# mrperkett/genome-kmers

Hardware: AMD Instinct MI355X
Metric: sorted 31-mers/sec end-to-end on 3.1 Gb synthetic genome; % HBM roofline (higher is better)
Workload: dtype u64

## Files before the change

genome-kmers_amd/csrc/gkm_msd.hip:

```cpp
#include <algorithm>
#include <cstdio>
#include <cstdlib>
#include <cstring>

#include "gkm_canon.h"
#include "gkm_internal.h"
#include "gkm_partition.h"
#include "gkm_swar.h"

namespace gkm {

constexpr int kGR = 8;
constexpr int kGRadix = 1 << kGR;
#ifndef GKM_PT
#define GKM_PT 1024
#endif
#ifndef GKM_PI
#define GKM_PI 11
#endif
constexpr int kPT = GKM_PT, kPI = GKM_PI;
constexpr int kWideL0 = 11, kWT = 512, kWI = 36;
constexpr int kPTile = kPT * kPI;
constexpr int kChunkTiles = 256;
constexpr int kBT = 512, kBI = 8, kBR = 8;
constexpr int kBT2 = 1024, kBR2 = 10;
constexpr int kBlockMax = kBT2 * kBI;
constexpr int kLocal = 6;
constexpr int kTiny = 8;
constexpr int kSmall = 24;
#ifndef GKM_WAVE_OCC8
#define GKM_WAVE_OCC8 4
#endif
constexpr int kWaveOcc4 = 6, kWaveOcc8 = GKM_WAVE_OCC8, kWaveOcc16 = 3;
#ifndef GKM_WAVE_R8
#define GKM_WAVE_R8 9
#endif
constexpr int kWaveR4 = 8, kWaveR8 = GKM_WAVE_R8, kWaveR16 = 10;
constexpr int kSmallLate = 96;
constexpr int kMaxLevels = 16;

__constant__ uint8_t c_code4_msd[256];
static bool g_msd_tables = false;

static hipError_t msd_tables() {
    if (g_msd_tables) return hipSuccess;
// ... 1120 lines not shown
            tile_hist[(f + i + u) * RADIX + d] = run;
            run += v[u];
        }
    }
    for (; i < nt; ++i) {
        const uint32_t v = tile_hist[(f + i) * RADIX + d];
        tile_hist[(f + i) * RADIX + d] = run;
        run += v;
    }
}

__device__ __forceinline__ uint32_t wave_append(bool flag, uint32_t *counter, int lane) {
    const uint64_t m = __ballot(flag);
    if (!m) return 0;
    const int leader = __ffsll((unsigned long long)m) - 1;
    uint32_t base = 0;
    if (lane == leader) base = atomicAdd(counter, (uint32_t)__popcll(m));
    base = __shfl(base, leader);
    const uint64_t lt_mask = (lane == 0) ? 0ull : (~0ull >> (64 - lane));
    return base + (uint32_t)__popcll(m & lt_mask);
}

enum { kCtrBig = 0, kCtrDone = 1, kCtrLoc = 2, kLists = kCtrLoc + kLocal, kCtrNbCopy = kLists, kCtrN = 8 + 2 };
enum { kSumTiles = kLists, kSumChunks = kLists + 1, kSumN = kLists + 2 };

__host__ __device__ inline uint32_t tiles_of(uint32_t len, uint32_t tile) { return (len + tile - 1) / tile; }
__host__ __device__ inline uint32_t chunks_of(uint32_t len, uint32_t tile, uint32_t ctiles) {
    return (tiles_of(len, tile) + ctiles - 1) / ctiles;
}

struct Lists {
    uint32_t *nb_start, *nb_len;
    uint32_t *dn_start, *dn_len;
    uint8_t *dn_par;
    uint2 *loc[kLocal];
    uint64_t *nb_pref;
    uint64_t *loc_pref[kLocal];
};

constexpr uint64_t kCompact = 1ull << 63;

__device__ __forceinline__ uint64_t compact_key(uint64_t pref, int hi, int B, uint32_t dig, uint32_t low) {
    const int rem = B - hi;
    return ((pref & ~kCompact) << rem) | ((uint64_t)dig << (rem - 8)) | (uint64_t)low;
}

__host__ __device__ constexpr uint32_t local_cap(int cls) {
// ... 22 lines not shown
        const uint2 le = local_entry(st, size, hi, parity);
        gmem(reinterpret_cast<uint64_t *>(L.loc[l - kCtrLoc]))[at] = ((uint64_t)le.y << 32) | le.x;
        if (L.loc_pref[l - kCtrLoc]) gmem(L.loc_pref[l - kCtrLoc])[at] = pref;
    }
}

__device__ __forceinline__ void route(uint32_t st, uint32_t size, int hi, int B, int parity, bool allow_big,
                                      const Lists &L, uint32_t *ctr, int lane) {
    const int li = size >= 1 ? list_of(size, hi, B, allow_big) : -1;
#pragma unroll
    for (int l = 0; l < kLists; ++l) {
        const uint32_t at = wave_append(li == l, &ctr[l], lane);
        if (li == l) put_entry(L, l, at, st, size, hi, parity);
    }
}

constexpr int kClassT = 1024;

__global__ __launch_bounds__(kClassT) void classify_kernel(const uint32_t *__restrict__ seg_base,
                                                           const uint32_t *__restrict__ seg_cnt, uint64_t nsub, int hi,
                                                           int B, int parity, Lists L, uint32_t *__restrict__ ctr,
                                                           unsigned long long *__restrict__ sums, uint32_t min_size,
                                                           const uint64_t *__restrict__ ppref, int pw, int compact,
                                                           uint32_t tile, uint32_t ctiles) {
    constexpr int NW = kClassT / 64;
    __shared__ uint32_t s_cnt[kLists][NW];
    __shared__ uint32_t s_elems[kLists][NW];
    __shared__ uint32_t s_base[kLists];
    __shared__ uint32_t s_tc[2][NW];
    const int tid = threadIdx.x, lane = tid & 63, wave = tid >> 6;
    const uint64_t i = (uint64_t)blockIdx.x * kClassT + tid;
    const uint32_t size = i < nsub ? seg_cnt[i] : 0, st = i < nsub ? seg_base[i] : 0;
    const int li = size >= min_size ? list_of(size, hi, B, true) : -1;
    bool f[kLists];
#pragma unroll
    for (int l = 0; l < kLists; ++l) f[l] = li == l;
    uint32_t below[kLists];
#pragma unroll
    for (int l = 0; l < kLists; ++l) {
        const uint64_t m = __ballot(f[l]);
        below[l] = lanes_below(m);
        uint32_t e = f[l] ? size : 0;
#pragma unroll
        for (int off = 32; off >= 1; off >>= 1) e += __shfl_xor(e, off);
        if (lane == 0) {
            s_cnt[l][wave] = (uint32_t)__popcll(m);
            s_elems[l][wave] = e;
        }
    }
    {
        uint32_t tl = li == kCtrBig ? tiles_of(size, tile) : 0, ch = li == kCtrBig ? chunks_of(size, tile, ctiles) : 0;
#pragma unroll
        for (int off = 32; off >= 1; off >>= 1) {
            tl += __shfl_xor(tl, off);
            ch += __shfl_xor(ch, off);
        }
        if (lane == 0) {
            s_tc[0][wave] = tl;
            s_tc[1][wave] = ch;
        }
    }
    __syncthreads();
    if (tid >= 64 && tid < 66) {
        unsigned long long t = 0;
        for (int w = 0; w < NW; ++w) t += s_tc[tid - 64][w];
        if (t) atomicAdd(&sums[kSumTiles + tid - 64], t);
    }
    if (tid < kLists) {
        uint32_t tot = 0;
        unsigned long long el = 0;
        for (int w = 0; w < NW; ++w) {
            tot += s_cnt[tid][w];
            el += s_elems[tid][w];
        }
        s_base[tid] = tot ? atomicAdd(&ctr[tid], tot) : 0;
        if (el) atomicAdd(&sums[tid], el);
    }
    __syncthreads();
    uint32_t at[kLists];
#pragma unroll
    for (int l = 0; l < kLists; ++l) {
        uint32_t pre = s_base[l];
        for (int w = 0; w < wave; ++w) pre += s_cnt[l][w];
        at[l] = pre + below[l];
    }
    uint64_t pref = 0;
// ... 841 lines not shown
}

__global__ __launch_bounds__(256) void uniform_flag_kernel(const uint32_t *__restrict__ bst,
                                                           const uint32_t *__restrict__ blen,
                                                           const uint64_t *__restrict__ keys,
                                                           uint32_t *__restrict__ mixed,
                                                           const uint32_t *__restrict__ nb_dev = nullptr,
                                                           uint32_t *__restrict__ nb_copy = nullptr) {
    if (nb_copy && blockIdx.x == 0 && blockIdx.y == 0 && threadIdx.x == 0) *nb_copy = *nb_dev;
    if (nb_dev && blockIdx.x >= *nb_dev) return;
    const uint64_t st = bst[blockIdx.x];
    const uint32_t len = blen[blockIdx.x];
    const uint64_t k0 = keys[st];
    uint64_t acc = 0;
    for (uint32_t e = blockIdx.y * 256 + threadIdx.x; e < len; e += gridDim.y * 256) acc |= keys[st + e] ^ k0;
    if (__syncthreads_or(acc != 0) && threadIdx.x == 0) atomicOr(&mixed[blockIdx.x], 1u);
}

__global__ __launch_bounds__(256) void route_uniform_kernel(const uint32_t *__restrict__ bst,
                                                            const uint32_t *__restrict__ blen,
                                                            const uint64_t *__restrict__ bpref, uint32_t nb,
                                                            const uint32_t *__restrict__ mixed, Lists L, int parity,
                                                            uint32_t *__restrict__ ctr,
                                                            unsigned long long *__restrict__ sums, uint32_t tile,
                                                            uint32_t ctiles, const uint32_t *__restrict__ nb_dev = nullptr) {
    if (nb_dev) nb = *nb_dev;
    for (uint32_t b = blockIdx.x * 256 + threadIdx.x; b < nb; b += gridDim.x * 256) {
        if (mixed[b]) {
            const uint32_t at = atomicAdd(&ctr[kCtrBig], 1u);
            put_entry(L, kCtrBig, at, bst[b], blen[b], 0, parity, bpref ? bpref[b] : 0);
            atomicAdd(&sums[kCtrBig], (unsigned long long)blen[b]);
            atomicAdd(&sums[kSumTiles], (unsigned long long)tiles_of(blen[b], tile));
            atomicAdd(&sums[kSumChunks], (unsigned long long)chunks_of(blen[b], tile, ctiles));
        } else {
            put_entry(L, kCtrDone, atomicAdd(&ctr[kCtrDone], 1u), bst[b], blen[b], 0, parity);
        }
    }
}

__global__ __launch_bounds__(256) void done_copy_kernel(const uint32_t *__restrict__ dn_start,
                                                        const uint32_t *__restrict__ dn_len,
                                                        const uint8_t *__restrict__ dn_par, const uint32_t *__restrict__ v1,
                                                        uint32_t *__restrict__ v0, const uint64_t *__restrict__ k1,
                                                        uint64_t *__restrict__ k0, uint8_t *__restrict__ heads) {
    const uint32_t s = blockIdx.x;
    const uint64_t st = dn_start[s];
    const uint32_t len = dn_len[s];
    const bool copy = dn_par[s];
    for (uint32_t i = blockIdx.y * 256 + threadIdx.x; i < len; i += gridDim.y * 256) {
        if (copy) v0[st + i] = v1[st + i];
        if (copy && k1) k0[st + i] = k1[st + i];
        heads[st + i] = i == 0;
    }
}

template <int BITS>
// ... 532 lines not shown
    int expand_big(int out) {
        if (cur_fmt != Fmt::Compact || nbig == 0) return GK_OK;
        hipLaunchKernelGGL(expand_compact_kernel, dim3(nbig, bucket_split(nbig)), dim3(256), 0, c->stream, big_start[cur_big],
                           big_len[cur_big], big_pref[cur_big], compact_hi, B, nd, c->keys[out], c->vals[out]);
        GK_TRY_HIP(c, hipGetLastError());
        return GK_OK;
    }

    int classify(uint64_t nsub, int hi, int parity, int bigsel, const uint32_t *base = nullptr,
                 const uint32_t *cnt = nullptr, uint32_t min_size = 1, const uint64_t *ppref = nullptr, int pw = 0,
                 int compact = 0, bool read = true) {
        if (!base) base = seg_base;
        if (!cnt) cnt = seg_cnt;
        for (int k = 0; k < kLocal; ++k)
            GK_TRY_HIP(c, grow_keep(c, kLocName[k][0], nloc[k] + nsub, nloc[k], &loc[k][0]));
        for (int k = 0; k < kLocal; ++k)
            GK_TRY_HIP(c, grow_keep(c, kLocPrefName[k], nloc[k] + nsub, nloc[k], &loc_pref[k]));
        if (int rc = grow_done(nsub)) return rc;
        GK_TRY_HIP(c, hipMemsetAsync(ctr + kCtrBig, 0, 4, c->stream));
        GK_TRY_HIP(c, hipMemsetAsync(sums, 0, 8 * kSumN, c->stream));
        timer_begin(c, "msd_classify", &slot);
        hipLaunchKernelGGL(classify_kernel, dim3((unsigned)((nsub + kClassT - 1) / kClassT)), dim3(kClassT), 0,
                           c->stream, base, cnt, nsub, hi, B, parity, lists(0, bigsel), ctr, sums, min_size, ppref, pw,
                           compact, (uint32_t)kPTile, ctiles);
        GK_TRY_HIP(c, hipGetLastError());
        timer_end(c, slot);
        return read ? classify_counts() : GK_OK;
    }

    int classify_counts() {
        int r = read_ctr();
        if (r != GK_OK) return r;
        for (int k = 0; k < kLocal; ++k) {
            nloc[k] = h[kCtrLoc + k];
            loc_elems[k] += hs[kCtrLoc + k];
        }
        ndone = h[kCtrDone];
        nbig = h[kCtrBig];
        big_elems = hs[kCtrBig];
        return GK_OK;
    }

    int route_uniform(int out, uint32_t nb, bool dev_count) {
        const uint32_t *nb_dev = dev_count ? ctr + kCtrBig : nullptr;
        uint32_t *nb_copy = dev_count ? ctr + kCtrNbCopy : nullptr;
        const unsigned split = bucket_split(nb);
        if (dev_count && cur_fmt == Fmt::Compact)
            hipLaunchKernelGGL(expand_compact_kernel, dim3(nb, split), dim3(256), 0, c->stream, big_start[cur_big],
                               big_len[cur_big], big_pref[cur_big], compact_hi, B, nd, c->keys[out], c->vals[out],
                               nb_dev);
        uint32_t *mixed;
        GK_TRY_HIP(c, scratch(c, "uni_mixed", nb, &mixed));
        GK_TRY_HIP(c, hipMemsetAsync(mixed, 0, 4ull * nb, c->stream));
        hipLaunchKernelGGL(uniform_flag_kernel, dim3(nb, split), dim3(256), 0, c->stream, big_start[cur_big],
                           big_len[cur_big], c->keys[out], mixed, nb_dev, nb_copy);
        if (!dev_count)
            if (int rc = grow_done(nb)) return rc;
        GK_TRY_HIP(c, hipMemsetAsync(ctr + kCtrBig, 0, 4, c->stream));
        GK_TRY_HIP(c, hipMemsetAsync(sums + kCtrBig, 0, 8, c->stream));
        GK_TRY_HIP(c, hipMemsetAsync(sums + kSumTiles, 0, 16, c->stream));
        hipLaunchKernelGGL(route_uniform_kernel, dim3(grid256_min1(nb)), dim3(256), 0, c->stream, big_start[cur_big],
                           big_len[cur_big], big_pref[cur_big], nb, mixed, lists(0, cur_big ^ 1), out, ctr, sums,
                           (uint32_t)kPTile, ctiles, nb_copy);
        GK_TRY_HIP(c, hipGetLastError());
        cur_big ^= 1;
        if (dev_count) return classify_counts();
        int r = read_ctr();
        if (r != GK_OK) return r;
        ndone = h[kCtrDone];
        nbig = h[kCtrBig];
        big_elems = hs[kCtrBig];
        return GK_OK;
    }

    bool few_big_elems(int level, uint64_t elems) const {
        return level >= 1 && elems * 64 <= std::max<uint64_t>(c->n, 1);
    }

    static bool reads(Fmt in, Fmt out) {
        switch (in) {
        case Fmt::Pairs: return out == Fmt::Compact;
        case Fmt::PackedL0: return out == Fmt::Pairs;
        default: return true;
        }
    }
    bool has_digits() const { return cur_fmt != Fmt::KeyStart; }

    template <int R>
    void level_launch(int hi, int nw, const uint32_t *t_start, const uint32_t *t_count, uint64_t T,
                      const uint64_t *kin, const uint32_t *vin, int out, bool count, Fmt ofmt) {
        if (count) {
            if (has_digits())
                hipLaunchKernelGGL(msd_count_nd_kernel<R>, dim3((unsigned)T), dim3(256), 0, c->stream, t_start,
                                   t_count, nd, tile_hist);
            else
                hipLaunchKernelGGL(msd_count_kernel<R>, dim3((unsigned)T), dim3(256), 0, c->stream, t_start, t_count,
                                   dig_at(B, hi, R), kin, tile_hist);
            return;
        }
        if (ofmt == Fmt::Compact) {
            const int rem = B - hi - R;
            NextDigits ndg{dig_at(B, hi + R, 8), nd};
            ndg.lowmask = (uint32_t)((1ull << (rem - 8)) - 1);
            if (cur_fmt == Fmt::Pairs)
                hipLaunchKernelGGL((msd_pipe_kernel<kPT, kPI, R, 4, true, 0, true>), dim3(pgrid), dim3(kPT), 0,
                                   c->stream, t_start, t_count, dig_at(B, hi, R), tile_hist, kin, vin, c->keys[out],
                                   c->vals[out], (uint32_t)T, n, ndg, lo16, c79_shi);
            else
                hipLaunchKernelGGL((msd_pipe_kernel<kPT, kPI, R, 4, true>), dim3(pgrid), dim3(kPT), 0, c->stream,
                                   t_start, t_count, dig_at(B, hi, R), tile_hist, kin, vin, c->keys[out],
                                   c->vals[out], (uint32_t)T, n, ndg);
            return;
        }
        if (ofmt == Fmt::Pairs) {
            NextDigits ndg{dig_at(B, hi + R, nw), nd};
            ndg.out16 = lo16;
            ndg.pshi = c79_shi;
            if (cur_fmt == Fmt::PackedL0) {
                ndg.in8 = nd_l0;
                hipLaunchKernelGGL((msd_pipe_kernel<kPT, kPI, R, 5, true, 0, 2>), dim3(pgrid), dim3(kPT), 0, c->stream,
                                   t_start, t_count, dig_at(B, hi, R), tile_hist, kin, vin, c->keys[out], c->vals[out],
                                   (uint32_t)T, n, ndg, lo16_l0, p88_shi);
                return;
            }
            hipLaunchKernelGGL((msd_pipe_kernel<kPT, kPI, R, 5, true>), dim3(pgrid), dim3(kPT), 0, c->stream, t_start,
                               t_count, dig_at(B, hi, R), tile_hist, kin, vin, c->keys[out], c->vals[out],
                               (uint32_t)T, n, ndg);
            return;
        }
        const NextDigits ndg{dig_at(B, hi + R, nw), nd};
        if (ofmt == Fmt::KeyStartDigit)
            hipLaunchKernelGGL((msd_pipe_kernel<kPT, kPI, R, 0, true>), dim3(pgrid), dim3(kPT), 0, c->stream, t_start,
                               t_count, dig_at(B, hi, R), tile_hist, kin, vin, c->keys[out], c->vals[out],
                               (uint32_t)T, n, ndg);
        else
            hipLaunchKernelGGL((msd_pipe_kernel<kPT, kPI, R, 0, false>), dim3(pgrid), dim3(kPT), 0, c->stream,
                               t_start, t_count, dig_at(B, hi, R), tile_hist, kin, vin, c->keys[out], c->vals[out],
                               (uint32_t)T, n, ndg);
    }

    void level_dispatch(int level, int hi, const uint32_t *t_start, const uint32_t *t_count, uint64_t T,
                        const uint64_t *kin, const uint32_t *vin, int out, bool count, Fmt ofmt) {
        const int w = width(level), nw = width(level + 1);
        if (w == 8) level_launch<8>(hi, nw, t_start, t_count, T, kin, vin, out, count, ofmt);
        else if (w == 7) level_launch<7>(hi, nw, t_start, t_count, T, kin, vin, out, count, ofmt);
        else level_launch<6>(hi, nw, t_start, t_count, T, kin, vin, out, count, ofmt);
    }

    Fmt level_format(int level, int hi, uint64_t elems, uint64_t nseg) const {
        const bool digits = nseg == 0 || (elems / nseg >> width(level)) >= (uint64_t)kBlockMax;
        const int rem = B - hi - width(level);
        if (phase == 0 && !digits && rem >= 9 && rem <= 40 && width(level + 1) == 8 && !no_compact())
            return Fmt::Compact;
        const uint64_t next_mean = nseg ? (elems / nseg >> width(level)) >> width(level + 1) : 0;
        const int rem2 = rem - width(level + 1);
        const bool force = opt("GKM_TEST_PAIRS") != nullptr;
        if (allow_c79 && cur_fmt != Fmt::Pairs && phase == 0 && rem >= 33 && rem <= 48 && !no_compact() &&
            (force || (digits && next_mean < (uint64_t)kBlockMax && rem2 >= 9 && rem2 <= 40 &&
                       width(level + 2) == 8 && width(level + 1) == 8)))
            return Fmt::Pairs;
        return digits ? Fmt::KeyStartDigit : Fmt::KeyStart;
    }

    int level_pass(int level, int hi, const uint32_t *t_start, const uint32_t *t_count, uint64_t T, uint64_t C,
                   const uint32_t *s_cfirst, const uint32_t *s_nchunks, const uint32_t *s_start, uint64_t nseg,
                   const uint64_t *kin, const uint32_t *vin, int out) {
        timer_begin(c, has_digits() ? "msd_count_nd" : "msd_count", &slot);
        timer_units(c, slot, big_elems);
        level_dispatch(level, hi, t_start, t_count, T, kin, vin, out, true, cur_fmt);
        GK_TRY_HIP(c, hipGetLastError());
        timer_end(c, slot);
        int rc = scan_offsets(width(level), C, s_cfirst, s_nchunks, s_start, nseg);
        if (rc != GK_OK) return rc;
        GK_TRY_HIP(c, scratch(c, "msd_nd", n + 64, &nd));
        const Fmt ofmt = level_format(level, hi, big_elems, nseg);
        compact_hi = hi + width(level);
        const int rem = B - hi - width(level);
        if (ofmt == Fmt::Pairs) {
            c79_shi = 64 - rem;
            GK_TRY_HIP(c, scratch(c, "msd_lo16", n + 64, &lo16));
        }
        if (!reads(cur_fmt, ofmt)) {
            if (cur_fmt == Fmt::PackedL0) {
                if (int rc = p88_detach()) return rc;
                hipLaunchKernelGGL(expand_p88_kernel, dim3((unsigned)nseg, bucket_split(nseg)), dim3(256), 0,
                                   c->stream, big_start[cur_big], big_len[cur_big], big_pref[cur_big], hi, B, p88_shi,
                                   const_cast<uint64_t *>(kin), lo16_l0, nd_l0, const_cast<uint32_t *>(vin));
            } else {
                hipLaunchKernelGGL(expand_pair_kernel, dim3((unsigned)nseg, bucket_split(nseg)), dim3(256), 0,
                                   c->stream, big_start[cur_big], big_len[cur_big], big_pref[cur_big], hi, B, c79_shi,
                                   const_cast<uint64_t *>(kin), lo16, const_cast<uint32_t *>(vin));
            }
            GK_TRY_HIP(c, hipGetLastError());
            cur_fmt = Fmt::KeyStartDigit;
        }
        timer_begin(c, ofmt == Fmt::Compact ? kPassNamesC[level & 7] : ofmt == Fmt::Pairs ? kPassNamesP[level & 7]
                                                                                          : kPassNames[level & 7],
                    &slot);
        timer_units(c, slot, big_elems);
        level_dispatch(level, hi, t_start, t_count, T, kin, vin, out, false, ofmt);
        GK_TRY_HIP(c, hipGetLastError());
        timer_end(c, slot);
        cur_fmt = ofmt;
        return GK_OK;
    }

    int expand_pair_locals(const uint64_t (&before)[kLocal], int out) {
        for (int k = 0; k < kLocal; ++k) {
            if (nloc[k] <= before[k]) continue;
            hipLaunchKernelGGL(expand_pair_list_kernel, dim3((unsigned)(nloc[k] - before[k])), dim3(256), 0,
                               c->stream, loc[k][0], loc_pref[k], (uint32_t)before[k], B, c79_shi, c->keys[out], lo16,
                               c->vals[out]);
            GK_TRY_HIP(c, hipGetLastError());
        }
        return GK_OK;
    }

    int first_level_from_pieces(const uint64_t *kin, const uint32_t *vin, const uint64_t *poff, const uint64_t *plen,
                                const uint32_t *pbucket, uint32_t np, int level = 1, int hi = kGR) {
        std::vector<uint32_t> ts, tc, cf, cn, scf, snc, sst;
        std::vector<uint64_t> spf;
        uint64_t out_base = 0;
        for (uint32_t i = 0; i < np;) {
            uint32_t j = i;
            uint64_t tot = 0;
            const uint64_t tile0 = ts.size();
            while (j < np && pbucket[j] == pbucket[i]) {
                for (uint64_t o = 0; o < plen[j]; o += kPTile) {
                    ts.push_back((uint32_t)(poff[j] + o));
                    tc.push_back((uint32_t)std::min<uint64_t>(kPTile, plen[j] - o));
                }
                tot += plen[j];
                ++j;
            }
            if (tot > 0) {
                const uint64_t nt = ts.size() - tile0;
                scf.push_back((uint32_t)cf.size());
                for (uint64_t t = 0; t < nt; t += ctiles) {
                    cf.push_back((uint32_t)(tile0 + t));
                    cn.push_back((uint32_t)std::min<uint64_t>(ctiles, nt - t));
                }
                snc.push_back((uint32_t)(cf.size() - scf.back()));
                sst.push_back((uint32_t)out_base);
                spf.push_back(pbucket[i]);
                out_base += tot;
            }
            i = j;
        }
        if (out_base != n) return fail(c, GK_E_ARG, "piece lengths do not add up to n");
        const uint64_t T = ts.size(), C = cf.size(), nseg = sst.size();
        if (nseg == 0) return GK_OK;
        int rc = tables(T, C, nseg);
        if (rc != GK_OK) return rc;
        uint32_t *t_start, *t_count, *s_cfirst, *s_nchunks, *s_st;
        GK_TRY_HIP(c, scratch(c, "t_start", T, &t_start));
        GK_TRY_HIP(c, scratch(c, "t_count", T, &t_count));
        GK_TRY_HIP(c, scratch(c, "s_cfirst", nseg, &s_cfirst));
        GK_TRY_HIP(c, scratch(c, "s_nchunks", nseg, &s_nchunks));
        GK_TRY_HIP(c, scratch(c, "s_pstart", nseg, &s_st));
        GK_TRY_HIP(c, hipMemcpyAsync(t_start, ts.data(), 4 * T, hipMemcpyHostToDevice, c->stream));
        GK_TRY_HIP(c, hipMemcpyAsync(t_count, tc.data(), 4 * T, hipMemcpyHostToDevice, c->stream));
        GK_TRY_HIP(c, hipMemcpyAsync(c_first, cf.data(), 4 * C, hipMemcpyHostToDevice, c->stream));
        GK_TRY_HIP(c, hipMemcpyAsync(c_ntiles, cn.data(), 4 * C, hipMemcpyHostToDevice, c->stream));
        GK_TRY_HIP(c, hipMemcpyAsync(s_cfirst, scf.data(), 4 * nseg, hipMemcpyHostToDevice, c->stream));
        GK_TRY_HIP(c, hipMemcpyAsync(s_nchunks, snc.data(), 4 * nseg, hipMemcpyHostToDevice, c->stream));
        GK_TRY_HIP(c, hipMemcpyAsync(s_st, sst.data(), 4 * nseg, hipMemcpyHostToDevice, c->stream));
        uint64_t *s_pref;
        GK_TRY_HIP(c, scratch(c, "s_ppref", nseg, &s_pref));
        GK_TRY_HIP(c, hipMemcpyAsync(s_pref, spf.data(), 8 * nseg, hipMemcpyHostToDevice, c->stream));
        GK_TRY_HIP(c, hipStreamSynchronize(c->stream));
        big_elems = n;
        if (!reads(cur_fmt, level_format(level, hi, n, nseg))) {
            if (int rd = p88_detach()) return rd;
            uint64_t *pdev;
            GK_TRY_HIP(c, scratch(c, "p88_pieces", 3 * np, &pdev));
            std::vector<uint64_t> hp(3 * (uint64_t)np);
            for (uint32_t j = 0; j < np; ++j) {
                hp[j] = poff[j];
                hp[np + j] = plen[j];
                hp[2 * (uint64_t)np + j] = pbucket[j];
            }
            GK_TRY_HIP(c, hipMemcpyAsync(pdev, hp.data(), 8 * hp.size(), hipMemcpyHostToDevice, c->stream));
            hipLaunchKernelGGL(expand_p88_pieces_kernel, dim3(np, bucket_split(np)), dim3(256), 0, c->stream, pdev,
                               np, hi, B, p88_shi, const_cast<uint64_t *>(kin), lo16_l0, nd_l0,
                               const_cast<uint32_t *>(vin));
            GK_TRY_HIP(c, hipGetLastError());
            GK_TRY_HIP(c, hipStreamSynchronize(c->stream));
            cur_fmt = Fmt::KeyStartDigit;
        }
        rc = level_pass(level, hi, t_start, t_count, T, C, s_cfirst, s_nchunks, s_st, nseg, kin, vin, 0);
        if (rc != GK_OK) return rc;
        cur_big = 0;
        uint64_t before[kLocal];
        for (int k = 0; k < kLocal; ++k) before[k] = nloc[k];
        rc = classify(nseg << width(level), hi + width(level), 0, cur_big, nullptr, nullptr, 1, s_pref, width(level),
                      cur_fmt == Fmt::Compact ? 1 : 0);
        if (rc == GK_OK && cur_fmt == Fmt::Pairs) rc = expand_pair_locals(before, 0);
        return rc == GK_OK ? expand_big(0) : rc;
    }

    unsigned tie_tiles() const { return (unsigned)std::max<uint64_t>((n + kTieTile - 1) / kTieTile, 1); }

    int tie_groups(const uint8_t *flags, uint32_t **g_start, uint32_t **g_len, uint64_t *ng,
                   uint32_t **tile_cnt = nullptr, uint32_t **tile_off = nullptr) {
        const unsigned ttiles = tie_tiles();
        uint32_t *cf, *cl, *of, *ol;
        GK_TRY_HIP(c, scratch(c, "tie_cnt_f", ttiles + 1, &cf));
        GK_TRY_HIP(c, scratch(c, "tie_cnt_l", ttiles + 1, &cl));
        GK_TRY_HIP(c, scratch(c, "tie_off_f", ttiles + 1, &of));
        GK_TRY_HIP(c, scratch(c, "tie_off_l", ttiles + 1, &ol));
        if (tile_cnt) *tile_cnt = cf;
        if (tile_off) *tile_off = of;
        hipLaunchKernelGGL(tie_bounds_kernel<false>, dim3(ttiles), dim3(256), 0, c->stream, flags, n, cf, cl, nullptr,
// ... 75 lines not shown
        nbig = 0;
        for (int k = 0; k < kLocal; ++k) nloc[k] = loc_elems[k] = 0;
        return sort_tied(g_start, g_len, ng);
    }

    int sort_groups(const uint8_t *flags, int bkey) {
        uint32_t *g_start, *g_len;
        uint64_t ng = 0;
        if (int rc = tie_groups(flags, &g_start, &g_len, &ng)) return rc;
        if (ng == 0) return GK_OK;
        B = bkey;
        phase = 1;
        return sort_tied(g_start, g_len, ng);
    }

    int levels(int level, int hi, int in) {
        while (nbig > 0) {
            const int out = in ^ 1;
            uint32_t *ntl, *nch, *tfirst, *cfirst;
            GK_TRY_HIP(c, scratch(c, "s_ntiles", nbig, &ntl));
            GK_TRY_HIP(c, scratch(c, "s_nchunks", nbig, &nch));
            GK_TRY_HIP(c, scratch(c, "s_tfirst", nbig, &tfirst));
            GK_TRY_HIP(c, scratch(c, "s_cfirst", nbig, &cfirst));
            const uint64_t T = hs[kSumTiles], C = hs[kSumChunks];
            if (nbig <= kSegScanMax && !opt("GKM_TEST_SEG_SCAN_MULTI")) {
                hipLaunchKernelGGL(seg_tiles_scan_kernel, dim3(1), dim3(1024), 0, c->stream, big_len[cur_big], nbig,
                                   (uint32_t)kPTile, ctiles, tfirst, cfirst, nch);
                GK_TRY_HIP(c, hipGetLastError());
            } else {
                hipLaunchKernelGGL(seg_counts_kernel, dim3(grid256_min1(nbig)), dim3(256), 0, c->stream, big_len[cur_big],
                                   nbig, (uint32_t)kPTile, ctiles, ntl, nch);
                GK_TRY_HIP(c, hipGetLastError());
                GK_TRY_HIP(c, scan_u32_exclusive_pair_launch(c, ntl, tfirst, nch, cfirst, nbig));
            }
            if (opt("GKM_TEST_CHECK_TILES")) {
                uint32_t last[4];
                GK_TRY_HIP(c, hipMemcpyAsync(&last[0], tfirst + nbig - 1, 4, hipMemcpyDeviceToHost, c->stream));
                GK_TRY_HIP(c, hipMemcpyAsync(&last[1], cfirst + nbig - 1, 4, hipMemcpyDeviceToHost, c->stream));
                GK_TRY_HIP(c, hipMemcpyAsync(&last[2], nch + nbig - 1, 4, hipMemcpyDeviceToHost, c->stream));
                GK_TRY_HIP(c, hipMemcpyAsync(&last[3], big_len[cur_big] + nbig - 1, 4, hipMemcpyDeviceToHost, c->stream));
                GK_TRY_HIP(c, hipStreamSynchronize(c->stream));
                if (last[0] + tiles_of(last[3], (uint32_t)kPTile) != T || last[1] + last[2] != C)
                    return fail(c, GK_E_HIP, "msd: level tile totals disagree with the bucket scan");
            }
            uint32_t *t_start, *t_count;
            GK_TRY_HIP(c, scratch(c, "t_start", T, &t_start));
            GK_TRY_HIP(c, scratch(c, "t_count", T, &t_count));
            int rc = tables(T, C, nbig);
            if (rc != GK_OK) return rc;
            hipLaunchKernelGGL(tile_table_kernel, dim3((unsigned)std::max<uint64_t>((std::max(T, C) + 255) / 256, 1)), dim3(256), 0,
                               c->stream, big_start[cur_big], big_len[cur_big], tfirst, cfirst, nbig,
                               (uint32_t)kPTile, (uint32_t)T, (uint32_t)C, ctiles, t_start, t_count, c_first, c_ntiles);
            const uint64_t in_big = big_elems;
            rc = level_pass(level, hi, t_start, t_count, T, C, cfirst, nch, big_start[cur_big], nbig, c->keys[in],
                            c->vals[in], out);
            if (rc != GK_OK) return rc;
            cur_big ^= 1;
            const bool pairs_out = cur_fmt == Fmt::Pairs;
            uint64_t before[kLocal];
            for (int k = 0; k < kLocal; ++k) before[k] = nloc[k];
            const uint64_t nsub = (uint64_t)nbig << width(level);
            const bool fuse = !pairs_out && few_big_elems(level, in_big) && !opt("GKM_NO_FUSED_UNIFORM");
            rc = classify(nsub, hi + width(level), out, cur_big, nullptr, nullptr, 1, big_pref[cur_big ^ 1],
                          width(level), cur_fmt == Fmt::Compact ? 1 : 0, !fuse);
            if (fuse) {
                const uint64_t bound = std::min<uint64_t>(nsub, in_big / ((uint64_t)kBlockMax + 1));
                if (rc == GK_OK) rc = bound ? route_uniform(out, (uint32_t)bound, true) : classify_counts();
            } else {
                if (rc == GK_OK && pairs_out) rc = expand_pair_locals(before, out);
                if (rc == GK_OK) rc = expand_big(out);
                if (rc == GK_OK && !pairs_out && nbig > 0 && few_big_elems(level, big_elems))
                    rc = route_uniform(out, nbig, false);
            }
            if (rc != GK_OK) return rc;
            ++level;
            hi += width(level - 1);
            in = out;
        }
// ... 649 lines not shown
```

genome-kmers_amd/csrc/gkm_partition.h:

```cpp
#pragma once

#include <hip/hip_runtime.h>
#include <stdint.h>

namespace gkm {

template <class T>
__device__ __forceinline__ __attribute__((address_space(1))) T *gmem(T *p) {
    return (__attribute__((address_space(1))) T *)p;
}
typedef __attribute__((address_space(1))) const uint64_t gu64;
typedef __attribute__((address_space(1))) const uint8_t gu8;
typedef __attribute__((address_space(1))) const uint32_t __attribute__((aligned(1))) gu32u;

__device__ __forceinline__ void lds_barrier() {
    __builtin_amdgcn_fence(__ATOMIC_RELEASE, "workgroup", "local");
    __builtin_amdgcn_s_barrier();
    __builtin_amdgcn_fence(__ATOMIC_ACQUIRE, "workgroup", "local");
}

constexpr int kVmcnt0 = 0x0F70;
constexpr int vmcnt_imm(int v) { return kVmcnt0 | (v & 15) | ((v >> 4) << 14); }

struct Dig {
// ... 335 lines not shown
            tp = t1;
        }
        for (int i = tid; i < SM::kWaves * RADIX; i += T) s_wc[i] = 0;
        if (tid < RADIX) s_toff[tid] = toff;
        lds_barrier();
        if (PROF && tid == 0) {
            const uint64_t t1 = clock64();
            atomicAdd(&prof[4], (unsigned long long)(t1 - tp));
            tp = t1;
        }
        bool valid[I];
#pragma unroll
        for (int i = 0; i < I; ++i) valid[i] = (uint32_t)(wave * (I * 64) + i * 64 + lane) < m;
        uint32_t slot[I];
        partition_stage<T, I, R, PROF>(key, val, valid, dl, s_raw, s_toff, s_wsum, s_start, slot, prof);
        if (PROF) tp = clock64();
        const uint32_t cnt = s_start[RADIX];
        const uint64_t seq = (uint64_t)t * (T * I);
        if (t + walk.step < walk.end) load(t + walk.step);
        partition_store<T, I, R, MODE>(dl, s_raw, s_toff, cnt, sink, kout, vout, seq);
    }
}

template <int T, int I>
struct PipeSmem {
    static constexpr int kTile = T * I;
    static constexpr int kWaves = T / 64;
    static constexpr int kValOff = (kTile + 2) * 8;
    static constexpr int kStage = kValOff + (kTile + 1) * 4;
};

struct NextDigits {
    Dig d;
    uint8_t *out;
    uint32_t lowmask = 0;
    uint16_t *out16 = nullptr;
    int pshi = 0;
    const uint8_t *in8 = nullptr;
};

__device__ __forceinline__ void unpack_pair(uint64_t a, uint32_t b16, int shi, uint64_t &key, uint32_t &val) {
    key = a >> shi;
    val = ((uint32_t)(a & ((1ull << shi) - 1)) << (32 - shi)) | b16;
}

template <int T, int I, int R, int MODE, bool ND>
__device__ __forceinline__ void pipe_store(int g, Dig d, const uint64_t *s_keys, const uint32_t *s_vals,
                                           const uint32_t *toff, uint32_t cnt, uint64_t sink,
                                           uint64_t *__restrict__ kout, uint32_t *__restrict__ vout,
                                           NextDigits nd, uint32_t base = 0) {
    const uint32_t s = min((uint32_t)(threadIdx.x + g * T), cnt - 1);
    const uint64_t k = s_keys[s];
    const uint32_t v = s_vals[s];
    const uint64_t o = cnt ? (uint64_t)(toff[dg_of(k, d)] + base + s) : sink;
    if (MODE == 4) {
        kout[o] = ((uint64_t)((uint32_t)k & nd.lowmask) << 32) | v;
        nd.out[o] = (uint8_t)dg_of(k, nd.d);
    } else if (MODE == 5) {
        const int shi = nd.pshi;
        kout[o] = ((k & ((1ull << (64 - shi)) - 1)) << shi) | (v >> (32 - shi));
        nd.out16[o] = (uint16_t)(v & ((1u << (32 - shi)) - 1));
        nd.out[o] = (uint8_t)dg_of(k, nd.d);
    } else if (MODE != 1 || o == 0xFFFFFFFFu) {
        kout[o] = k;
        vout[o] = v;
        if (ND) nd.out[o] = (uint8_t)dg_of(k, nd.d);
    }
}

template <int T, int I, int R = 8, int MODE = 0, bool ND = false, int PRE_ = 0, int INP = 0>
__global__ __launch_bounds__(T) void msd_pipe_kernel(const uint32_t *__restrict__ t_start,
                                                     const uint32_t *__restrict__ t_count, Dig dl,
                                                     const uint32_t *__restrict__ tile_off,
                                                     const uint64_t *__restrict__ kin, const uint32_t *__restrict__ vin,
                                                     uint64_t *__restrict__ kout, uint32_t *__restrict__ vout,
                                                     uint32_t ntiles, uint64_t sink, NextDigits nd = {},
                                                     const uint16_t *__restrict__ in16 = nullptr, int in_shi = 0) {
    static_assert(INP == 0 || MODE == 4 || MODE == 5, "packed-pair input keeps only the unsorted key bits");
    using SM = PipeSmem<T, I>;
    constexpr int NW = SM::kWaves;
    constexpr int TILE = SM::kTile;
    constexpr int PRE = PRE_ ? PRE_ : (I + 2) / 3;
    constexpr int RADIX = 1 << R;
    static_assert(T >= RADIX, "one thread per digit");
    __shared__ __attribute__((aligned(16))) unsigned char s_stage[SM::kStage];
    __shared__ uint32_t s_wc[NW * RADIX];
    __shared__ uint32_t s_toff[2][RADIX];
    __shared__ uint32_t s_start[RADIX + 1];
    __shared__ uint32_t s_wsum[RADIX / 64 > 0 ? RADIX / 64 : 1];
    uint64_t *s_keys = reinterpret_cast<uint64_t *>(s_stage);
    uint32_t *s_vals = reinterpret_cast<uint32_t *>(s_stage + SM::kValOff);
    const int tid = threadIdx.x, lane = tid & 63, wave = tid >> 6;
    const TileWalk walk(ntiles);
    uint64_t key[I];
    uint32_t val[I], m = 0, toff = 0;
    auto load = [&](uint32_t t) {
        toff = tile_off[(uint64_t)t * RADIX + (tid & (RADIX - 1))];
        const uint64_t b = t_start[t];
        m = t_count[t];
        uint32_t q0 = wave * (I * 64) + lane;
        asm volatile("" : "+v"(q0));
#pragma unroll
        for (int i = 0; i < I; ++i) {
            const uint64_t e = b + min(q0 + i * 64, m - 1);
            if (INP == 1) {
                key[i] = kin[e];
                val[i] = in16[e];
            } else if (INP == 2) {
                key[i] = kin[e];
                val[i] = in16[e] | ((uint32_t)nd.in8[e] << 16);
            } else {
                key[i] = kin[e];
                val[i] = vin[e];
            }
        }
    };
    uint32_t pcnt = 0;
    int cur = 0;
    if (walk.first < walk.end) load(walk.first);
    __builtin_amdgcn_s_waitcnt(kVmcnt0);
    for (uint32_t t = walk.first; t < walk.end; t += walk.step) {
        uint32_t *wc = s_wc + wave * RADIX;
#pragma unroll
        for (int u = 0; u < (RADIX + 63) / 64; ++u)
            if (u * 64 + lane < RADIX) wc[u * 64 + lane] = 0;
        if (tid < RADIX) s_toff[cur][tid] = toff;
        const uint32_t *ptoff = s_toff[cur ^ 1];
#pragma unroll
        for (int g = 0; g < PRE; ++g) pipe_store<T, I, R, MODE, ND>(g, dl, s_keys, s_vals, ptoff, pcnt, sink, kout, vout, nd);
        bool valid[I];
        uint32_t dig[I], rank[I];
#pragma unroll
        for (int i = 0; i < I; ++i) {
            valid[i] = (uint32_t)(wave * (I * 64) + i * 64 + lane) < m;
            if (INP == 1) unpack_pair(key[i], val[i], in_shi, key[i], val[i]);
            if (INP == 2) {
                const uint64_t top = (uint64_t)(val[i] >> 16) << (64 - in_shi);
                unpack_pair(key[i], val[i] & 0xFFFFu, in_shi, key[i], val[i]);
                key[i] |= top;
            }
            dig[i] = dg_of(key[i], dl);
            rank[i] = rank_atomic(wc, dig[i], valid[i]);
            if (PRE + i < I) pipe_store<T, I, R, MODE, ND>(PRE + i, dl, s_keys, s_vals, ptoff, pcnt, sink, kout, vout, nd);
        }
        lds_barrier();
        uint32_t total = 0, incl = 0;
        if (tid < RADIX) {
#pragma unroll
            for (int w = 0; w < NW; ++w) {
                const uint32_t v = s_wc[w * RADIX + tid];
                s_wc[w * RADIX + tid] = total;
                total += v;
            }
            incl = wave_incl_scan(total);
            if (lane == 63) s_wsum[wave] = incl;
        }
        lds_barrier();
        if (tid < RADIX) {
            uint32_t pre = 0;
            for (int w = 0; w < wave; ++w) pre += s_wsum[w];
            const uint32_t st = pre + incl - total;
            s_start[tid] = st;
            s_toff[cur][tid] -= st;
            if (tid == RADIX - 1) s_start[RADIX] = pre + incl;
        }
        lds_barrier();
#pragma unroll
        for (int i = 0; i < I; ++i) {
            const uint32_t sl = valid[i] ? s_start[dig[i]] + wc[dig[i]] + rank[i] : (uint32_t)TILE;
            s_keys[sl] = key[i];
            s_vals[sl] = val[i];
        }
        pcnt = s_start[RADIX];
        lds_barrier();
        if (t + walk.step < walk.end) load(t + walk.step);
        cur ^= 1;
    }
    if (walk.first < walk.end) {
        const uint32_t *ptoff = s_toff[cur ^ 1];
#pragma unroll
        for (int g = 0; g < I; ++g) pipe_store<T, I, R, MODE, ND>(g, dl, s_keys, s_vals, ptoff, pcnt, sink, kout, vout, nd);
    }
}

}
```

Measured before the change: 44.37 billion.

## Enlarge compact-format MSD tiles and pack staging with run-table offsets

Adds a second tile size used when the level outputs the compact format. Tile and chunk totals are computed for both sizes in classify and route, and the host picks the set matching the level's output format. In the packed MODE 4 pipe kernel, the 64-bit key and 8-bit aux are built before staging, so LDS holds one byte of aux per element instead of four. The per-tile digit offset becomes a run-length table found by popcount, so the staging fits larger tiles (14 items per thread instead of 11). The aim is fewer tiles and less LDS per element in compact passes, at the cost of extra atomics to build the table, a serial fill loop per digit, and a 16-bit limit on the tile count.

```diff
diff --git a/genome-kmers_amd/csrc/gkm_msd.hip b/genome-kmers_amd/csrc/gkm_msd.hip
--- a/genome-kmers_amd/csrc/gkm_msd.hip
+++ b/genome-kmers_amd/csrc/gkm_msd.hip
@@ -20,7 +20,14 @@
 #endif
 constexpr int kPT = GKM_PT, kPI = GKM_PI;
 constexpr int kWideL0 = 11, kWT = 512, kWI = 36;
-constexpr int kPTile = kPT * kPI;
+#ifndef GKM_PI_COMPACT
+#define GKM_PI_COMPACT 14
+#endif
+constexpr int kPIC = GKM_PI_COMPACT;
+constexpr int kTileKinds = 2;
+__host__ __device__ constexpr uint32_t tile_of_kind(int kind) {
+    return (uint32_t)(kPT * (kind == 0 ? kPI : kPIC));
+}
 constexpr int kChunkTiles = 256;
 constexpr int kBT = 512, kBI = 8, kBR = 8;
 constexpr int kBT2 = 1024, kBR2 = 10;
@@ -1187,7 +1194,7 @@
 }
 
 enum { kCtrBig = 0, kCtrDone = 1, kCtrLoc = 2, kLists = kCtrLoc + kLocal, kCtrNbCopy = kLists, kCtrN = 8 + 2 };
-enum { kSumTiles = kLists, kSumChunks = kLists + 1, kSumN = kLists + 2 };
+enum { kSumTiles = kLists, kSumChunks = kLists + 1, kSumN = kLists + 2 * kTileKinds };
 
 __host__ __device__ inline uint32_t tiles_of(uint32_t len, uint32_t tile) { return (len + tile - 1) / tile; }
 __host__ __device__ inline uint32_t chunks_of(uint32_t len, uint32_t tile, uint32_t ctiles) {
@@ -1256,12 +1263,12 @@
                                                            int B, int parity, Lists L, uint32_t *__restrict__ ctr,
                                                            unsigned long long *__restrict__ sums, uint32_t min_size,
                                                            const uint64_t *__restrict__ ppref, int pw, int compact,
-                                                           uint32_t tile, uint32_t ctiles) {
+                                                           uint32_t ctiles) {
     constexpr int NW = kClassT / 64;
     __shared__ uint32_t s_cnt[kLists][NW];
     __shared__ uint32_t s_elems[kLists][NW];
     __shared__ uint32_t s_base[kLists];
-    __shared__ uint32_t s_tc[2][NW];
+    __shared__ uint32_t s_tc[2 * kTileKinds][NW];
     const int tid = threadIdx.x, lane = tid & 63, wave = tid >> 6;
     const uint64_t i = (uint64_t)blockIdx.x * kClassT + tid;
     const uint32_t size = i < nsub ? seg_cnt[i] : 0, st = i < nsub ? seg_base[i] : 0;
@@ -1282,7 +1289,9 @@
             s_elems[l][wave] = e;
         }
     }
-    {
+#pragma unroll
+    for (int kind = 0; kind < kTileKinds; ++kind) {
+        const uint32_t tile = tile_of_kind(kind);
         uint32_t tl = li == kCtrBig ? tiles_of(size, tile) : 0, ch = li == kCtrBig ? chunks_of(size, tile, ctiles) : 0;
 #pragma unroll
         for (int off = 32; off >= 1; off >>= 1) {
@@ -1290,12 +1299,12 @@
             ch += __shfl_xor(ch, off);
         }
         if (lane == 0) {
-            s_tc[0][wave] = tl;
-            s_tc[1][wave] = ch;
+            s_tc[2 * kind][wave] = tl;
+            s_tc[2 * kind + 1][wave] = ch;
         }
     }
     __syncthreads();
-    if (tid >= 64 && tid < 66) {
+    if (tid >= 64 && tid < 64 + 2 * kTileKinds) {
         unsigned long long t = 0;
         for (int w = 0; w < NW; ++w) t += s_tc[tid - 64][w];
         if (t) atomicAdd(&sums[kSumTiles + tid - 64], t);
@@ -2183,7 +2192,7 @@
                                                             const uint64_t *__restrict__ bpref, uint32_t nb,
                                                             const uint32_t *__restrict__ mixed, Lists L, int parity,
                                                             uint32_t *__restrict__ ctr,
-                                                            unsigned long long *__restrict__ sums, uint32_t tile,
+                                                            unsigned long long *__restrict__ sums,
                                                             uint32_t ctiles, const uint32_t *__restrict__ nb_dev = nullptr) {
     if (nb_dev) nb = *nb_dev;
     for (uint32_t b = blockIdx.x * 256 + threadIdx.x; b < nb; b += gridDim.x * 256) {
@@ -2191,8 +2200,12 @@
             const uint32_t at = atomicAdd(&ctr[kCtrBig], 1u);
             put_entry(L, kCtrBig, at, bst[b], blen[b], 0, parity, bpref ? bpref[b] : 0);
             atomicAdd(&sums[kCtrBig], (unsigned long long)blen[b]);
-            atomicAdd(&sums[kSumTiles], (unsigned long long)tiles_of(blen[b], tile));
-            atomicAdd(&sums[kSumChunks], (unsigned long long)chunks_of(blen[b], tile, ctiles));
+#pragma unroll
+            for (int kind = 0; kind < kTileKinds; ++kind) {
+                const uint32_t tile = tile_of_kind(kind);
+                atomicAdd(&sums[kSumTiles + 2 * kind], (unsigned long long)tiles_of(blen[b], tile));
+                atomicAdd(&sums[kSumChunks + 2 * kind], (unsigned long long)chunks_of(blen[b], tile, ctiles));
+            }
         } else {
             put_entry(L, kCtrDone, atomicAdd(&ctr[kCtrDone], 1u), bst[b], blen[b], 0, parity);
         }
@@ -2771,7 +2784,7 @@
         timer_begin(c, "msd_classify", &slot);
         hipLaunchKernelGGL(classify_kernel, dim3((unsigned)((nsub + kClassT - 1) / kClassT)), dim3(kClassT), 0,
                            c->stream, base, cnt, nsub, hi, B, parity, lists(0, bigsel), ctr, sums, min_size, ppref, pw,
-                           compact, (uint32_t)kPTile, ctiles);
+                           compact, ctiles);
         GK_TRY_HIP(c, hipGetLastError());
         timer_end(c, slot);
         return read ? classify_counts() : GK_OK;
@@ -2807,10 +2820,10 @@
             if (int rc = grow_done(nb)) return rc;
         GK_TRY_HIP(c, hipMemsetAsync(ctr + kCtrBig, 0, 4, c->stream));
         GK_TRY_HIP(c, hipMemsetAsync(sums + kCtrBig, 0, 8, c->stream));
-        GK_TRY_HIP(c, hipMemsetAsync(sums + kSumTiles, 0, 16, c->stream));
+        GK_TRY_HIP(c, hipMemsetAsync(sums + kSumTiles, 0, 16 * kTileKinds, c->stream));
         hipLaunchKernelGGL(route_uniform_kernel, dim3(grid256_min1(nb)), dim3(256), 0, c->stream, big_start[cur_big],
                            big_len[cur_big], big_pref[cur_big], nb, mixed, lists(0, cur_big ^ 1), out, ctr, sums,
-                           (uint32_t)kPTile, ctiles, nb_copy);
+                           ctiles, nb_copy);
         GK_TRY_HIP(c, hipGetLastError());
         cur_big ^= 1;
         if (dev_count) return classify_counts();
@@ -2852,11 +2865,11 @@
             NextDigits ndg{dig_at(B, hi + R, 8), nd};
             ndg.lowmask = (uint32_t)((1ull << (rem - 8)) - 1);
             if (cur_fmt == Fmt::Pairs)
-                hipLaunchKernelGGL((msd_pipe_kernel<kPT, kPI, R, 4, true, 0, true>), dim3(pgrid), dim3(kPT), 0,
+                hipLaunchKernelGGL((msd_pipe_kernel<kPT, kPIC, R, 4, true, 0, 1>), dim3(pgrid), dim3(kPT), 0,
                                    c->stream, t_start, t_count, dig_at(B, hi, R), tile_hist, kin, vin, c->keys[out],
                                    c->vals[out], (uint32_t)T, n, ndg, lo16, c79_shi);
             else
-                hipLaunchKernelGGL((msd_pipe_kernel<kPT, kPI, R, 4, true>), dim3(pgrid), dim3(kPT), 0, c->stream,
+                hipLaunchKernelGGL((msd_pipe_kernel<kPT, kPIC, R, 4, true>), dim3(pgrid), dim3(kPT), 0, c->stream,
                                    t_start, t_count, dig_at(B, hi, R), tile_hist, kin, vin, c->keys[out],
                                    c->vals[out], (uint32_t)T, n, ndg);
             return;
@@ -2896,6 +2909,7 @@
         else level_launch<6>(hi, nw, t_start, t_count, T, kin, vin, out, count, ofmt);
     }
 
+    static int level_tile_kind(Fmt ofmt) { return ofmt == Fmt::Compact ? 1 : 0; }
     Fmt level_format(int level, int hi, uint64_t elems, uint64_t nseg) const {
         const bool digits = nseg == 0 || (elems / nseg >> width(level)) >= (uint64_t)kBlockMax;
         const int rem = B - hi - width(level);
@@ -2913,7 +2927,7 @@
 
     int level_pass(int level, int hi, const uint32_t *t_start, const uint32_t *t_count, uint64_t T, uint64_t C,
                    const uint32_t *s_cfirst, const uint32_t *s_nchunks, const uint32_t *s_start, uint64_t nseg,
-                   const uint64_t *kin, const uint32_t *vin, int out) {
+                   const uint64_t *kin, const uint32_t *vin, int out, Fmt ofmt) {
         timer_begin(c, has_digits() ? "msd_count_nd" : "msd_count", &slot);
         timer_units(c, slot, big_elems);
         level_dispatch(level, hi, t_start, t_count, T, kin, vin, out, true, cur_fmt);
@@ -2922,7 +2936,6 @@
         int rc = scan_offsets(width(level), C, s_cfirst, s_nchunks, s_start, nseg);
         if (rc != GK_OK) return rc;
         GK_TRY_HIP(c, scratch(c, "msd_nd", n + 64, &nd));
-        const Fmt ofmt = level_format(level, hi, big_elems, nseg);
         compact_hi = hi + width(level);
         const int rem = B - hi - width(level);
         if (ofmt == Fmt::Pairs) {
@@ -2969,15 +2982,25 @@
                                 const uint32_t *pbucket, uint32_t np, int level = 1, int hi = kGR) {
         std::vector<uint32_t> ts, tc, cf, cn, scf, snc, sst;
         std::vector<uint64_t> spf;
+        uint64_t nbuckets = 0;
+        for (uint32_t i = 0; i < np;) {
+            uint32_t j = i;
+            uint64_t tot = 0;
+            for (; j < np && pbucket[j] == pbucket[i]; ++j) tot += plen[j];
+            nbuckets += tot > 0;
+            i = j;
+        }
+        const Fmt ofmt = level_format(level, hi, n, nbuckets);
+        const uint64_t tile = tile_of_kind(level_tile_kind(ofmt));
         uint64_t out_base = 0;
         for (uint32_t i = 0; i < np;) {
             uint32_t j = i;
             uint64_t tot = 0;
             const uint64_t tile0 = ts.size();
             while (j < np && pbucket[j] == pbucket[i]) {
-                for (uint64_t o = 0; o < plen[j]; o += kPTile) {
+                for (uint64_t o = 0; o < plen[j]; o += tile) {
                     ts.push_back((uint32_t)(poff[j] + o));
-                    tc.push_back((uint32_t)std::min<uint64_t>(kPTile, plen[j] - o));
+                    tc.push_back((uint32_t)std::min<uint64_t>(tile, plen[j] - o));
                 }
                 tot += plen[j];
                 ++j;
@@ -3019,7 +3042,7 @@
         GK_TRY_HIP(c, hipMemcpyAsync(s_pref, spf.data(), 8 * nseg, hipMemcpyHostToDevice, c->stream));
         GK_TRY_HIP(c, hipStreamSynchronize(c->stream));
         big_elems = n;
-        if (!reads(cur_fmt, level_format(level, hi, n, nseg))) {
+        if (!reads(cur_fmt, ofmt)) {
             if (int rd = p88_detach()) return rd;
             uint64_t *pdev;
             GK_TRY_HIP(c, scratch(c, "p88_pieces", 3 * np, &pdev));
@@ -3037,7 +3060,7 @@
             GK_TRY_HIP(c, hipStreamSynchronize(c->stream));
             cur_fmt = Fmt::KeyStartDigit;
         }
-        rc = level_pass(level, hi, t_start, t_count, T, C, s_cfirst, s_nchunks, s_st, nseg, kin, vin, 0);
+        rc = level_pass(level, hi, t_start, t_count, T, C, s_cfirst, s_nchunks, s_st, nseg, kin, vin, 0, ofmt);
         if (rc != GK_OK) return rc;
         cur_big = 0;
         uint64_t before[kLocal];
@@ -3159,14 +3182,17 @@
             GK_TRY_HIP(c, scratch(c, "s_nchunks", nbig, &nch));
             GK_TRY_HIP(c, scratch(c, "s_tfirst", nbig, &tfirst));
             GK_TRY_HIP(c, scratch(c, "s_cfirst", nbig, &cfirst));
-            const uint64_t T = hs[kSumTiles], C = hs[kSumChunks];
+            const Fmt ofmt = level_format(level, hi, big_elems, nbig);
+            const int kind = level_tile_kind(ofmt);
+            const uint32_t tile = tile_of_kind(kind);
+            const uint64_t T = hs[kSumTiles + 2 * kind], C = hs[kSumChunks + 2 * kind];
             if (nbig <= kSegScanMax && !opt("GKM_TEST_SEG_SCAN_MULTI")) {
                 hipLaunchKernelGGL(seg_tiles_scan_kernel, dim3(1), dim3(1024), 0, c->stream, big_len[cur_big], nbig,
-                                   (uint32_t)kPTile, ctiles, tfirst, cfirst, nch);
+                                   tile, ctiles, tfirst, cfirst, nch);
                 GK_TRY_HIP(c, hipGetLastError());
             } else {
                 hipLaunchKernelGGL(seg_counts_kernel, dim3(grid256_min1(nbig)), dim3(256), 0, c->stream, big_len[cur_big],
-                                   nbig, (uint32_t)kPTile, ctiles, ntl, nch);
+                                   nbig, tile, ctiles, ntl, nch);
                 GK_TRY_HIP(c, hipGetLastError());
                 GK_TRY_HIP(c, scan_u32_exclusive_pair_launch(c, ntl, tfirst, nch, cfirst, nbig));
             }
@@ -3177,7 +3203,7 @@
                 GK_TRY_HIP(c, hipMemcpyAsync(&last[2], nch + nbig - 1, 4, hipMemcpyDeviceToHost, c->stream));
                 GK_TRY_HIP(c, hipMemcpyAsync(&last[3], big_len[cur_big] + nbig - 1, 4, hipMemcpyDeviceToHost, c->stream));
                 GK_TRY_HIP(c, hipStreamSynchronize(c->stream));
-                if (last[0] + tiles_of(last[3], (uint32_t)kPTile) != T || last[1] + last[2] != C)
+                if (last[0] + tiles_of(last[3], tile) != T || last[1] + last[2] != C)
                     return fail(c, GK_E_HIP, "msd: level tile totals disagree with the bucket scan");
             }
             uint32_t *t_start, *t_count;
@@ -3187,10 +3213,10 @@
             if (rc != GK_OK) return rc;
             hipLaunchKernelGGL(tile_table_kernel, dim3((unsigned)std::max<uint64_t>((std::max(T, C) + 255) / 256, 1)), dim3(256), 0,
                                c->stream, big_start[cur_big], big_len[cur_big], tfirst, cfirst, nbig,
-                               (uint32_t)kPTile, (uint32_t)T, (uint32_t)C, ctiles, t_start, t_count, c_first, c_ntiles);
+                               tile, (uint32_t)T, (uint32_t)C, ctiles, t_start, t_count, c_first, c_ntiles);
             const uint64_t in_big = big_elems;
             rc = level_pass(level, hi, t_start, t_count, T, C, cfirst, nch, big_start[cur_big], nbig, c->keys[in],
-                            c->vals[in], out);
+                            c->vals[in], out, ofmt);
             if (rc != GK_OK) return rc;
             cur_big ^= 1;
             const bool pairs_out = cur_fmt == Fmt::Pairs;
diff --git a/genome-kmers_amd/csrc/gkm_partition.h b/genome-kmers_amd/csrc/gkm_partition.h
--- a/genome-kmers_amd/csrc/gkm_partition.h
+++ b/genome-kmers_amd/csrc/gkm_partition.h
@@ -381,12 +381,34 @@
     }
 }
 
-template <int T, int I>
+template <int MODE>
+struct PipeElem {
+    static constexpr bool kPacked = MODE == 4;
+    static constexpr int kAuxBytes = MODE == 4 ? 1 : 4;
+};
+template <int BYTES>
+struct AuxType {
+    typedef uint32_t type;
+};
+template <>
+struct AuxType<1> {
+    typedef uint8_t type;
+};
+
+template <int T, int I, int MODE = 0, int R = 8>
 struct PipeSmem {
     static constexpr int kTile = T * I;
     static constexpr int kWaves = T / 64;
+    static constexpr int kRadix = 1 << R;
+    static constexpr bool kPacked = PipeElem<MODE>::kPacked;
     static constexpr int kValOff = (kTile + 2) * 8;
-    static constexpr int kStage = kValOff + (kTile + 1) * 4;
+    static constexpr int kStage = kValOff + ((kTile + 1) * PipeElem<MODE>::kAuxBytes + 15) / 16 * 16;
+    static constexpr int kTabWords = kTile / 16;
+    static_assert(kTile % 16 == 0 && kTabWords <= T, "one thread per run-table word");
+    static constexpr int kTotal = kStage + kWaves * kRadix * 4 + (kPacked ? 1 : 2) * kRadix * 4 + (kRadix + 1) * 4 +
+                                  (kRadix / 64 > 0 ? kRadix / 64 : 1) * 4 +
+                                  (kPacked ? (kTabWords + 1) * 4 : 0);
+    static_assert(kTotal <= 160 * 1024, "the tile's staging does not fit the LDS of a CU");
 };
 
 struct NextDigits {
@@ -403,19 +425,34 @@
     val = ((uint32_t)(a & ((1ull << shi) - 1)) << (32 - shi)) | b16;
 }
 
+__device__ __forceinline__ void pack_compact(uint64_t k, uint32_t v, const NextDigits &nd, uint64_t &pk, uint32_t &aux) {
+    pk = ((uint64_t)((uint32_t)k & nd.lowmask) << 32) | v;
+    aux = dg_of(k, nd.d);
+}
+
+__device__ __forceinline__ uint32_t runtab_offset(const uint32_t *tab, const uint32_t *ctoff, uint32_t s) {
+    const uint32_t e = tab[s >> 4];
+    const uint32_t r = (e >> 16) + (uint32_t)__popc(e & ((2u << (s & 15)) - 2u) & 0xFFFFu);
+    return ctoff[r] + s;
+}
+
 template <int T, int I, int R, int MODE, bool ND>
-__device__ __forceinline__ void pipe_store(int g, Dig d, const uint64_t *s_keys, const uint32_t *s_vals,
-                                           const uint32_t *toff, uint32_t cnt, uint64_t sink,
+__device__ __forceinline__ void pipe_store(int g, Dig d, const uint64_t *s_keys,
+                                           const typename AuxType<PipeElem<MODE>::kAuxBytes>::type *s_aux,
+                                           const uint32_t *toff, const uint32_t *tab, uint32_t cnt, uint64_t sink,
                                            uint64_t *__restrict__ kout, uint32_t *__restrict__ vout,
                                            NextDigits nd, uint32_t base = 0) {
     const uint32_t s = min((uint32_t)(threadIdx.x + g * T), cnt - 1);
     const uint64_t k = s_keys[s];
-    const uint32_t v = s_vals[s];
+    const uint32_t v = s_aux[s];
+    if (MODE == 4) {
+        const uint64_t o = cnt ? (uint64_t)runtab_offset(tab, toff, s) : sink;
+        kout[o] = k;
+        nd.out[o] = (uint8_t)v;
+        return;
+    }
     const uint64_t o = cnt ? (uint64_t)(toff[dg_of(k, d)] + base + s) : sink;
-    if (MODE == 4) {
-        kout[o] = ((uint64_t)((uint32_t)k & nd.lowmask) << 32) | v;
-        nd.out[o] = (uint8_t)dg_of(k, nd.d);
-    } else if (MODE == 5) {
+    if (MODE == 5) {
         const int shi = nd.pshi;
         kout[o] = ((k & ((1ull << (64 - shi)) - 1)) << shi) | (v >> (32 - shi));
         nd.out16[o] = (uint16_t)(v & ((1u << (32 - shi)) - 1));
@@ -436,19 +473,26 @@
                                                      uint32_t ntiles, uint64_t sink, NextDigits nd = {},
                                                      const uint16_t *__restrict__ in16 = nullptr, int in_shi = 0) {
     static_assert(INP == 0 || MODE == 4 || MODE == 5, "packed-pair input keeps only the unsorted key bits");
-    using SM = PipeSmem<T, I>;
+    using SM = PipeSmem<T, I, MODE, R>;
+    using Aux = typename AuxType<PipeElem<MODE>::kAuxBytes>::type;
+    constexpr bool PK = SM::kPacked;
     constexpr int NW = SM::kWaves;
     constexpr int TILE = SM::kTile;
     constexpr int PRE = PRE_ ? PRE_ : (I + 2) / 3;
     constexpr int RADIX = 1 << R;
+    constexpr int DW = RADIX / 64 > 0 ? RADIX / 64 : 1;
+    constexpr int NTAB = SM::kTabWords;
     static_assert(T >= RADIX, "one thread per digit");
+    static_assert(!PK || TILE < 65536, "the packed scan carries the tile's element count in 16 bits");
+    static_assert(!PK || R <= 8, "digit and rank of a packed item share a register");
     __shared__ __attribute__((aligned(16))) unsigned char s_stage[SM::kStage];
     __shared__ uint32_t s_wc[NW * RADIX];
-    __shared__ uint32_t s_toff[2][RADIX];
+    __shared__ uint32_t s_toff[PK ? 1 : 2][RADIX];
     __shared__ uint32_t s_start[RADIX + 1];
-    __shared__ uint32_t s_wsum[RADIX / 64 > 0 ? RADIX / 64 : 1];
+    __shared__ uint32_t s_wsum[DW];
+    __shared__ uint32_t s_tab[PK ? NTAB + 1 : 1];
     uint64_t *s_keys = reinterpret_cast<uint64_t *>(s_stage);
-    uint32_t *s_vals = reinterpret_cast<uint32_t *>(s_stage + SM::kValOff);
+    Aux *s_vals = reinterpret_cast<Aux *>(s_stage + SM::kValOff);
     const int tid = threadIdx.x, lane = tid & 63, wave = tid >> 6;
     const TileWalk walk(ntiles);
     uint64_t key[I];
@@ -476,6 +520,10 @@
     };
     uint32_t pcnt = 0;
     int cur = 0;
+    if (PK) {
+        for (int i = tid; i < NTAB + 1; i += T) s_tab[i] = 0;
+        lds_barrier();
+    }
     if (walk.first < walk.end) load(walk.first);
     __builtin_amdgcn_s_waitcnt(kVmcnt0);
     for (uint32_t t = walk.first; t < walk.end; t += walk.step) {
@@ -483,10 +531,11 @@
 #pragma unroll
         for (int u = 0; u < (RADIX + 63) / 64; ++u)
             if (u * 64 + lane < RADIX) wc[u * 64 + lane] = 0;
-        if (tid < RADIX) s_toff[cur][tid] = toff;
-        const uint32_t *ptoff = s_toff[cur ^ 1];
-#pragma unroll
-        for (int g = 0; g < PRE; ++g) pipe_store<T, I, R, MODE, ND>(g, dl, s_keys, s_vals, ptoff, pcnt, sink, kout, vout, nd);
+        if (!PK && tid < RADIX) s_toff[cur][tid] = toff;
+        const uint32_t *ptoff = s_toff[PK ? 0 : cur ^ 1];
+#pragma unroll
+        for (int g = 0; g < PRE; ++g)
+            pipe_store<T, I, R, MODE, ND>(g, dl, s_keys, s_vals, ptoff, s_tab, pcnt, sink, kout, vout, nd);
         bool valid[I];
         uint32_t dig[I], rank[I];
 #pragma unroll
@@ -499,11 +548,14 @@
                 key[i] |= top;
             }
             dig[i] = dg_of(key[i], dl);
+            if (MODE == 4) pack_compact(key[i], val[i], nd, key[i], val[i]);
             rank[i] = rank_atomic(wc, dig[i], valid[i]);
-            if (PRE + i < I) pipe_store<T, I, R, MODE, ND>(PRE + i, dl, s_keys, s_vals, ptoff, pcnt, sink, kout, vout, nd);
+            if (PK) dig[i] |= rank[i] << 8;
+            if (PRE + i < I)
+                pipe_store<T, I, R, MODE, ND>(PRE + i, dl, s_keys, s_vals, ptoff, s_tab, pcnt, sink, kout, vout, nd);
         }
         lds_barrier();
-        uint32_t total = 0, incl = 0;
+        uint32_t total = 0, incl = 0, sv = 0;
         if (tid < RADIX) {
 #pragma unroll
             for (int w = 0; w < NW; ++w) {
@@ -511,24 +563,44 @@
                 s_wc[w * RADIX + tid] = total;
                 total += v;
             }
-            incl = wave_incl_scan(total);
+            sv = PK ? total | (total ? 1u << 16 : 0u) : total;
+            incl = wave_incl_scan(sv);
             if (lane == 63) s_wsum[wave] = incl;
         }
+        if (PK && tid < NTAB) s_tab[tid] = 0;
         lds_barrier();
         if (tid < RADIX) {
-            uint32_t pre = 0;
-            for (int w = 0; w < wave; ++w) pre += s_wsum[w];
-            const uint32_t st = pre + incl - total;
-            s_start[tid] = st;
-            s_toff[cur][tid] -= st;
-            if (tid == RADIX - 1) s_start[RADIX] = pre + incl;
+            uint32_t pre = 0, all = 0;
+#pragma unroll
+            for (int w = 0; w < DW; ++w) {
+                const uint32_t v = s_wsum[w];
+                pre += w < wave ? v : 0u;
+                all += v;
+            }
+            if (PK) {
+                const uint32_t ex = pre + incl - sv;
+                const uint32_t st = ex & 0xFFFFu, r = ex >> 16;
+                s_start[tid] = st;
+                if (tid == RADIX - 1) s_start[RADIX] = all & 0xFFFFu;
+                if (total) {
+                    s_toff[0][r] = toff - st;
+                    atomicOr(&s_tab[st >> 4], 1u << (st & 15));
+                    for (uint32_t w = (st + 15) >> 4; (w << 4) < st + total; ++w) atomicOr(&s_tab[w], r << 16);
+                }
+            } else {
+                const uint32_t st = pre + incl - total;
+                s_start[tid] = st;
+                s_toff[cur][tid] -= st;
+                if (tid == RADIX - 1) s_start[RADIX] = all;
+            }
         }
         lds_barrier();
 #pragma unroll
         for (int i = 0; i < I; ++i) {
-            const uint32_t sl = valid[i] ? s_start[dig[i]] + wc[dig[i]] + rank[i] : (uint32_t)TILE;
+            const uint32_t dg = PK ? dig[i] & 0xFFu : dig[i], rk = PK ? dig[i] >> 8 : rank[i];
+            const uint32_t sl = valid[i] ? s_start[dg] + wc[dg] + rk : (uint32_t)TILE;
             s_keys[sl] = key[i];
-            s_vals[sl] = val[i];
+            s_vals[sl] = (Aux)val[i];
         }
         pcnt = s_start[RADIX];
         lds_barrier();
@@ -536,10 +608,11 @@
         cur ^= 1;
     }
     if (walk.first < walk.end) {
-        const uint32_t *ptoff = s_toff[cur ^ 1];
-#pragma unroll
-        for (int g = 0; g < I; ++g) pipe_store<T, I, R, MODE, ND>(g, dl, s_keys, s_vals, ptoff, pcnt, sink, kout, vout, nd);
-    }
-}
-
-}
+        const uint32_t *ptoff = s_toff[PK ? 0 : cur ^ 1];
+#pragma unroll
+        for (int g = 0; g < I; ++g)
+            pipe_store<T, I, R, MODE, ND>(g, dl, s_keys, s_vals, ptoff, s_tab, pcnt, sink, kout, vout, nd);
+    }
+}
+
+}
```

New measurement: 44.60 billion, median of 5. Within noise of the previous version (+0.5%).
